# introlab/rtabmap

Measured on AMD Instinct MI355X. Metric: loop-closure candidates/sec (49k vocab, 100k signatures, 500 desc/frame), higher is better.
Workload: dtype f32; 1 GPU; SURF-64 fp32 brute-force 2-NN (49k words) + NNDR + TF-IDF likelihood (100000 signatures x 500 words, Zipf), 500 desc/frame, 1 frame/step; world_size_observed=1, collective_backend=none, parallelism=1 GPU, last_frame_top_candidate_ok=True

## Files before the change

### rtabmap_amd/csrc/bf16_filter_body.cuh

```cuda
#pragma once

constexpr int BF_KEEP = 2;
constexpr int BF_QW = 128;
constexpr int BF_NG = BF_QW / 32;
constexpr int BF_QB = BF_QW * MF_WAVES;
constexpr int BF_TILE_F = 32 * 64;
constexpr size_t BF_LDS_BYTES = (size_t)(MF_WAVES * 4 + 2) * BF_TILE_F * 4 + (size_t)MF_STRIP_TILES * 64 * 4;
typedef __bf16 bf16x8_t __attribute__((ext_vector_type(8)));

template <bool HI = false>
__device__ __forceinline__ void dma_tile_part(const float* __restrict__ base, int n_rows, int t, int lane, float* __restrict__ lds_slot,
                                              int i0, int i1) {
    for (int i = i0; i < i1; ++i) {
        const int p = i * 64 + lane;
        const int r = p >> 4, cpos = p & 15;
        const int c = cpos ^ (r & 15);
        if (HI && c >= 8) continue;
        const int row = min(t * 32 + r, n_rows - 1);
        __builtin_amdgcn_global_load_lds((const __attribute__((address_space(1))) void*)(base + (size_t)row * 64 + c * 4),
                                         (__attribute__((address_space(3))) void*)(lds_slot + i * 256), 16, 0, 0);
    }
}
typedef _Float16 f16x8_t __attribute__((ext_vector_type(8)));
template <int M>
// ... 449 lines not shown
            const int i = 2 * wave + j;
            if (half == 0 && (tile0 + i) * 32 + col >= lo_rows)
                asm volatile("ds_write_b32 %0, %1" ::"v"((uint32_t)(uintptr_t)(__attribute__((address_space(3))) void*)(s_aug + i * 64 + lane)),
                             "v"(__int_as_float(0x7f800000)) : "memory");
        }
        asm volatile("s_waitcnt lgkmcnt(0)" ::: "memory");
    }
    __builtin_amdgcn_s_barrier();
    MF_STAMP(1);
    int32_t k0[NG], k1[NG], k2[NG];
#pragma unroll
    for (int g = 0; g < NG; ++g) { k0[g] = MF_KEY_NONE; k1[g] = MF_KEY_NONE; k2[g] = MF_KEY_NONE; }
    f32x16 p0, p1;
    for (int t = tile0; t < tile1; ++t) {
        const int ti = t - tile0;
        if (ti == 2) {
            asm volatile("s_waitcnt vmcnt(0)" ::: "memory");
            __builtin_amdgcn_s_barrier();
        }
        uint4 ah[4], al[4];
        float aug;
        {
            const float* slot = s_dyn + (size_t)ti * BF_TILE_F;
            const uint32_t base = (uint32_t)(uintptr_t)(__attribute__((address_space(3))) const void*)(slot + col * 64);
            uint32_t addr[8];
            uint4 av[8];
#pragma unroll
            for (int v = 0; v < 4; ++v) {
                addr[v] = a_chunk_addr(base, 4 * half + v, col);
                addr[4 + v] = a_chunk_addr(base, 8 + 4 * half + v, col);
// ... 62 lines not shown
#pragma unroll
        for (int m = 0; m < 4; ++m)
            *reinterpret_cast<float4*>(xs + (size_t)ql * 32 + (((2 * m + half) ^ (ql & 7)) << 2)) = make_float4(c[g][4 * m], c[g][4 * m + 1], c[g][4 * m + 2], c[g][4 * m + 3]);
    }
    asm volatile("s_waitcnt lgkmcnt(0)" ::: "memory");
#pragma unroll 4
    for (int it = 0; it < QW / 8; ++it) {
        const int ql = it * 8 + (lane >> 3), ck = lane & 7;
        const int qi = q0 + ql;
        const float4 v = *reinterpret_cast<const float4*>(xs + (size_t)ql * 32 + ((ck ^ (ql & 7)) << 2));
        if (qi < nq) *reinterpret_cast<float4*>(x + (size_t)qi * ld + t * 32 + 4 * ck) = v;
    }
}

constexpr size_t BF_LDS_BYTES_P = (size_t)(MF_WAVES * 4 + 2) * BF_TILE_F * 4 + (size_t)2 * MF_STRIP_TILES * 64 * 4;
__device__ const float g_aug_inf[2] = {__builtin_inff(), 1.0f};
template <int M>
__device__ __forceinline__ void bf_request_strip(const float* __restrict__ vocab_bf, const float* __restrict__ row_norm, int n_rows, int bx,
                                                 int tiles_per_block, int n_tiles, int lane, int wave, int col, int half, float* slots, float* aug_dst) {
    constexpr int DPW = 8 / MF_WAVES;
    const int tile0 = bx * tiles_per_block;
    const int tile1 = min(tile0 + tiles_per_block, n_tiles);
#pragma unroll
    for (int i = 0; i < MF_STRIP_TILES; ++i) {
        const int t = min(tile0 + i, max(tile1 - 1, tile0));
        dma_tile_part<M == 1>(vocab_bf, n_rows, t, lane, slots + (size_t)i * BF_TILE_F, DPW * wave, DPW * wave + DPW);
    }
    if (wave == 0) {
#pragma unroll
        for (int i = 0; i < MF_STRIP_TILES; ++i) {
            const int t = min(tile0 + i, max(tile1 - 1, tile0));
            const float* src = t * 32 + col >= n_rows ? g_aug_inf + half : row_norm + 2 * (size_t)(t * 32 + col) + half;
            __builtin_amdgcn_global_load_lds((const __attribute__((address_space(1))) void*)src,
                                             (__attribute__((address_space(3))) void*)(aug_dst + i * 64), 4, 0, 0);
        }
    }
}
__device__ __forceinline__ void bf_wait_all_but_request(int wave) {
    constexpr int DPW = 8 / MF_WAVES;
    if (wave == 0) asm volatile("s_waitcnt vmcnt(%0)" :: "n"(MF_STRIP_TILES * DPW + MF_STRIP_TILES) : "memory");
    else asm volatile("s_waitcnt vmcnt(%0)" :: "n"(MF_STRIP_TILES * DPW) : "memory");
}
__device__ __forceinline__ void bf_lds_barrier() { asm volatile("s_waitcnt lgkmcnt(0)\n\ts_barrier" ::: "memory"); }
template <int M>
__device__ __forceinline__ void knn_bf16_filter_body_p(float* s_dyn, int bid, const float* __restrict__ vocab_bf, const float* __restrict__ row_norm,
                                                       int n_rows, const float* __restrict__ queries, int nq, int qpad,
                                                       int tiles_per_block, int n_blocks, int px, StripRecord* __restrict__ records, const SelfdistJob& sd,
                                                       const int32_t* __restrict__ n_lo = nullptr) {
    if (n_lo) n_rows = min(n_rows, max(n_lo[0], 1));
    constexpr int NG = BF_NG;
    constexpr int KH = 32;
    constexpr int NW = MF_WAVES;
    constexpr int QW = BF_QW;
    constexpr int DPW = 8 / NW;
    const int n_fwg = px * ((nq + BF_QB - 1) / BF_QB);
    if (bid >= n_fwg) { selfdist_tile(sd, bid - n_fwg, s_dyn); return; }
    const int fb = bid;
    const int bx0 = fb % px, by = fb / px;
    const int n_my = (n_blocks - bx0 + px - 1) / px;
    const int lane = threadIdx.x & 63;
    const int wave = __builtin_amdgcn_readfirstlane(threadIdx.x >> 6);
    const int col = lane & 31, half = lane >> 5;
    const int q0 = by * BF_QB + wave * QW;
    float* s_q = s_dyn + (size_t)wave * NG * BF_TILE_F;
    float* s_tile = s_dyn + (size_t)NW * NG * BF_TILE_F;
    float* s_aug = s_tile + 2 * BF_TILE_F;
    const int n_tiles = (n_rows + 31) / 32;
    {
        const int tile0 = bx0 * tiles_per_block;
        const int tile1 = min(tile0 + tiles_per_block, n_tiles);
#pragma unroll
        for (int g = 0; g < NG; ++g) dma_a_tile<KH>(queries, nq, q0 / 32 + g, lane, s_q + g * BF_TILE_F);
        float augs[MF_STRIP_TILES];
#pragma unroll
        for (int i = 0; i < MF_STRIP_TILES; ++i) {
            const int t = min(tile0 + i, max(tile1 - 1, tile0));
            augs[i] = t * 32 + col >= n_rows ? g_aug_inf[half] : row_norm[2 * (size_t)(t * 32 + col) + half];
        }
        if (tile0 < tile1) {
            dma_tile_part<M == 1>(vocab_bf, n_rows, tile0, lane, s_tile, DPW * wave, DPW * wave + DPW);
            dma_tile_part<M == 1>(vocab_bf, n_rows, min(tile0 + 1, tile1 - 1), lane, s_tile + BF_TILE_F, DPW * wave, DPW * wave + DPW);
        }
        asm volatile("s_waitcnt vmcnt(0)" ::: "memory");
        if (wave == 0) {
#pragma unroll
            for (int i = 0; i < MF_STRIP_TILES; ++i) s_aug[i * 64 + lane] = augs[i];
        }
    }
    uint4 bh[NG][4], bl[NG][4];
    float b_aug[NG];
#pragma unroll
    for (int g = 0; g < NG; ++g) split_query_group<M>(s_q + g * BF_TILE_F, col, half, bh[g], bl[g], b_aug[g]);
    __syncthreads();
    {
        const int tile0 = bx0 * tiles_per_block;
        const int tile1 = min(tile0 + tiles_per_block, n_tiles);
        for (int t = tile0 + 2; t < tile1; ++t)
            dma_tile_part<M == 1>(vocab_bf, n_rows, t, lane, s_dyn + (size_t)(t - tile0 - 2) * BF_TILE_F, DPW * wave, DPW * wave + DPW);
    }
    if (n_my > 1) bf_request_strip<M>(vocab_bf, row_norm, n_rows, bx0 + px, tiles_per_block, n_tiles, lane, wave, col, half,
                                   s_dyn + (size_t)8 * BF_TILE_F, s_aug + MF_STRIP_TILES * 64);
    for (int s = 0; s < n_my; ++s) {
        const int bx = bx0 + s * px;
        const int tile0 = bx * tiles_per_block;
        const int tile1 = min(tile0 + tiles_per_block, n_tiles);
        if (s > 0) {
            if (s + 1 < n_my) bf_wait_all_but_request(wave); else asm volatile("s_waitcnt vmcnt(0)" ::: "memory");
            bf_lds_barrier();
        }
        int32_t k0[NG], k1[NG], k2[NG];
#pragma unroll
        for (int g = 0; g < NG; ++g) { k0[g] = MF_KEY_NONE; k1[g] = MF_KEY_NONE; k2[g] = MF_KEY_NONE; }
        f32x16 p0, p1;
        const float* aug_s = s_aug + (s & 1) * (MF_STRIP_TILES * 64);
        for (int t = tile0; t < tile1; ++t) {
            const int ti = t - tile0;
            if (s == 0 && ti == 2) {
                if (n_my > 1) bf_wait_all_but_request(wave); else asm volatile("s_waitcnt vmcnt(0)" ::: "memory");
                bf_lds_barrier();
            }
            uint4 ah[4], al[4];
            float aug;
            {
                const float* slot = s == 0 ? (ti < 2 ? s_tile + ti * BF_TILE_F : s_dyn + (size_t)(ti - 2) * BF_TILE_F)
                                           : s_dyn + (size_t)(((s & 1) ? 8 : 0) + ti) * BF_TILE_F;
                const uint32_t base = (uint32_t)(uintptr_t)(__attribute__((address_space(3))) const void*)(slot + col * 64);
                uint32_t addr[8];
                uint4 av[8];
#pragma unroll
                for (int v = 0; v < 4; ++v) {
                    addr[v] = a_chunk_addr(base, 4 * half + v, col);
                    addr[4 + v] = a_chunk_addr(base, 8 + 4 * half + v, col);
                }
                lds_read_ops<M>(addr, av, (uint32_t)(uintptr_t)(__attribute__((address_space(3))) const void*)(aug_s + ti * 64 + lane), aug);
#pragma unroll
                for (int v = 0; v < 4; ++v) { ah[v] = av[v]; al[v] = av[4 + v]; }
            }
            tile_trip<M>(t == tile0, (uint32_t)ti, ah, al, aug, bh, bl, b_aug, p0, p1, k0, k1, k2);
        }
        if (tile0 < tile1) flush_pending(p0, p1, (uint32_t)(tile1 - 1 - tile0), k0, k1, k2);
#pragma unroll
        for (int g = 0; g < NG; ++g) merge_store_keys(k0[g], k1[g], k2[g], half, q0 + g * 32 + col, qpad, bx, records);
        if (s + 2 < n_my) {
            bf_lds_barrier();
            bf_request_strip<M>(vocab_bf, row_norm, n_rows, bx0 + (s + 2) * px, tiles_per_block, n_tiles, lane, wave, col, half,
                             s_dyn + (size_t)((s & 1) ? 8 : 0) * BF_TILE_F, s_aug + (s & 1) * (MF_STRIP_TILES * 64));
        }
    }
}
```

### rtabmap_amd/csrc/frame_pipeline.hip

```cpp
#include "engine_impl.h"

#include <algorithm>
#include <chrono>
#include <cstring>

using namespace lcd;

namespace {
struct FrameHostTimer {
    lcd_engine* h; std::chrono::steady_clock::time_point t0;
    explicit FrameHostTimer(lcd_engine* e) : h(e), t0(std::chrono::steady_clock::now()) {}
    ~FrameHostTimer() { h->frame_host_ns += std::chrono::duration_cast<std::chrono::nanoseconds>(std::chrono::steady_clock::now() - t0).count(); h->frame_calls += 1; }
};
struct HostLap {
    lcd_engine* h; std::chrono::steady_clock::time_point t;
    explicit HostLap(lcd_engine* e) : h(e), t(std::chrono::steady_clock::now()) {}
    void lap(int i) { const auto n = std::chrono::steady_clock::now(); h->host_prof[i] += std::chrono::duration_cast<std::chrono::nanoseconds>(n - t).count(); t = n; }
};
struct FrameShape { bool incremental, together; int ld, bw; };
inline FrameShape frame_shape(const lcd_frame_args& a) {
    const bool incremental = (a.flags & LCD_Q_INCREMENTAL) != 0;
    const int ld = (a.q + 63) / 64 * 64;
    return FrameShape{incremental, incremental && (a.flags & LCD_Q_NEW_WORDS_COMPARED) != 0, ld, ld / 32};
}
// ... 119 lines not shown
    PipeKnn& k = *kp;
    const lcd_frame_args& a = f.a;
    const int q = a.q;
    FramePipeline::FrameScratch& sc = h->pipe.scratch(f);
    const auto [incremental, together, ld, bw] = frame_shape(a);
    const int64_t rows_bound = f.chained ? h->applog.rows_ub(h->n_rows) : h->n_rows;
    const int64_t plan_rows = f.chained ? h->applog.rows_plan(f.vseq, h->n_rows) : h->n_rows;
    if (plan_rows > 0x7FFFFFF0ll) return h->fail(LCD_ERR_UNSUPPORTED, "lcd_frame_dev: more than 2^31 rows");
    k.plan = knn_bf16_plan_pipelined(q, (int)plan_rows, together ? knn_selfdist_wgs(q) : 0, h->filter_units);
    k.plan.f16 = h->f16();
    if (h->strip_tiles > 0 && plan_rows > 0) {
        const int n_tiles = (int)((plan_rows + 31) / 32);
        k.plan.tiles_per_block = h->strip_tiles; k.plan.n_blocks = (n_tiles + h->strip_tiles - 1) / h->strip_tiles; k.plan.one_strip = 1;
        k.plan.f16 = h->f16();
    }
    if (f_sh && !knn_bf16_persistent(k.plan) && plan_rows < (int64_t)SHADOW_ROW_BASE) {
        const FramePipeline::FrameScratch& ss = h->pipe.scratch(*f_sh);
        k.plan.n_shadow = 1;
        k.sh_bf = ss.d_shadow_bf.p; k.sh_norm = ss.d_shadow_norm.as<float>(); k.sh_rows = (f_sh->a.q + 63) / 64 * 64;
        k.sh_mask = ss.d_newmask.as<uint32_t>(); k.sh_q = f_sh->a.q;
        k.sh_ld = k.sh_rows;
        LCD_HIP(h, ring_reserve(h, f.set, &FramePipeline::FrameScratch::d_cross, (size_t)q * k.sh_ld * 4));
        k.sh_x = sc.d_cross.as<float>();
    }
    {
        size_t bytes = knn_bf16_partial_bytes(k.plan), want = 0;
        if (f.chained) {
            bytes = std::max(bytes, knn_bf16_partial_bytes(knn_bf16_plan_pipelined(q, (int)(rows_bound + 8 * (int64_t)q), together ? knn_selfdist_wgs(q) : 0, h->filter_units)));
            want = knn_bf16_partial_bytes(knn_bf16_plan_pipelined(q, (int)std::min<int64_t>(rows_bound + rows_bound / 2 + 65536, 0x7FFFFF00ll), together ? knn_selfdist_wgs(q) : 0, h->filter_units));
        }
        LCD_HIP(h, ring_reserve_grow(h, f.set, &FramePipeline::FrameScratch::d_partial2, bytes, want));
// ... 368 lines not shown
```

### rtabmap_amd/csrc/knn_mfma_kernels.hip

```cpp
#include <hip/hip_ext.h>
#include "lcd_kernels.h"
#include "rowpar_body.cuh"
#include "shard_body.cuh"
#include "frame_tail_body.cuh"
#include "score_body.cuh"

#include <algorithm>
#include <cstdlib>

namespace lcd {
namespace {

typedef float f32x16 __attribute__((ext_vector_type(16)));
constexpr int MF_BLOCK = 256;
constexpr int MF_WAVES = 4;
constexpr int MF_KEEP = 4;

__global__ void row_norm_kernel(const float* __restrict__ vocab, const int32_t* __restrict__ row_id, int first, int n, int dim,
                                float* __restrict__ aug, uint32_t* __restrict__ norm_max_bits) {
    const int r = first + blockIdx.x * blockDim.x + threadIdx.x;
    if (r >= first + n) return;
    float s = __int_as_float(0x7f800000);
    if (row_id[r] != 0) {
        s = 0.0f;
// ... 186 lines not shown
        top3_push32(k00, k01, k02, strip_key(p0[r], mask, base | (uint32_t)r));
        top3_push32(k10, k11, k12, strip_key(p1[r], mask, base | (uint32_t)r));
        __builtin_amdgcn_sched_barrier(0);
    }
}

constexpr int MF_NG = 4;
#ifdef LCD_MFMA_TIMING
__device__ unsigned long long g_mf_timing[4 * 4096];
#define MF_STAMP(i) do { if (lane == 0) g_mf_timing[4 * (((blockIdx.y * gridDim.x + blockIdx.x) & 1023) * MF_WAVES + wave) + (i)] = __builtin_amdgcn_s_memrealtime(); } while (0)
__device__ unsigned long long g_mf_timing2[8 * 4096];
#define MF_STAMP2(i) do { if (lane == 0 && (i) < 8) { g_mf_timing2[8 * (((blockIdx.y * gridDim.x + blockIdx.x) & 1023) * MF_WAVES + wave) + (i)] = __builtin_amdgcn_s_memrealtime(); } } while (0)
#else
#define MF_STAMP(i) do { } while (0)
#define MF_STAMP2(i) do { } while (0)
#endif

template <int DIM>
__global__ __launch_bounds__(MF_BLOCK, 1) void knn_mfma_filter_kernel(const float* __restrict__ vocab, const float* __restrict__ row_norm, int n_rows,
                                                                     const float* __restrict__ queries, int nq, int qpad, int tiles_per_block,
                                                                     uint64_t* __restrict__ partial_keys, uint32_t* __restrict__ partial_lmin) {
    constexpr int NG = MF_NG;
    constexpr int KH = DIM / 2;
    constexpr int QW = NG * 32;
    const int lane = threadIdx.x & 63;
    const int wave = __builtin_amdgcn_readfirstlane(threadIdx.x >> 6);
    const int col = lane & 31, half = lane >> 5;
    const int q0 = blockIdx.y * QW;
    MF_STAMP(0);

// ... 100 lines not shown
            for (int i = 0; i < MF_KEEP; ++i) partial_keys[((size_t)qi * gridDim.x + blockIdx.x) * MF_KEEP + i] = keep[i];
            partial_lmin[(size_t)qi * gridDim.x + blockIdx.x] = lmin;
        }
    }
    MF_STAMP(3);
}


#include "bf16_filter_body.cuh"

template <int M>
__global__ __launch_bounds__(256) void knn_bf16_filter_kernel_p(const float* __restrict__ vocab_bf, const float* __restrict__ row_norm, int n_rows,
                                                                const float* __restrict__ queries, int nq, int qpad, int tiles_per_block, int n_blocks,
                                                                int px, StripRecord* __restrict__ records, SelfdistJob sd) {
    extern __shared__ __attribute__((aligned(16))) float s_dyn_p[];
    knn_bf16_filter_body_p<M>(s_dyn_p, (int)blockIdx.x, vocab_bf, row_norm, n_rows, queries, nq, qpad, tiles_per_block, n_blocks, px, records, sd);
}

template <int M>
__global__ __launch_bounds__(MF_WAVES * 64) void knn_bf16_filter_kernel(const float* __restrict__ vocab_bf, const float* __restrict__ row_norm,
                                                                      int n_rows, const float* __restrict__ queries, int nq, int qpad,
                                                                      int tiles_per_block, int n_blocks, StripRecord* __restrict__ records,
                                                                      SelfdistJob sd) {
    extern __shared__ __attribute__((aligned(16))) float s_dyn_f[];
    knn_bf16_filter_body<M>(s_dyn_f, (int)blockIdx.x, vocab_bf, row_norm, n_rows, queries, nq, qpad, tiles_per_block, n_blocks, records, sd);
}

#include "rerank_body.cuh"

template <int DIM, int KEEP, bool LAST_KEY_BOUNDS, bool BF16>
__global__ __launch_bounds__(MF_BLOCK) void knn_mfma_rerank_kernel(KeptKeys<BF16> kk, int n_blocks, int nq,
// ... 34 lines not shown
__device__ unsigned long long g_a_timing[2 * 4096];
#define A_STAMP(i) do { __builtin_amdgcn_s_barrier(); if (threadIdx.x == 0 && blockIdx.x < 4096) g_a_timing[2 * blockIdx.x + (i)] = __builtin_amdgcn_s_memrealtime(); } while (0)
#else
#define A_STAMP(i) do { } while (0)
#endif
template <bool PERSISTENT, int M>
__device__ __forceinline__ void frame_a_body(float* s_dyn, const FilterArgs& f, int px, const TailRoles& tr, const ResolveArgs& r, const FwArgs& a,
                                             const RetireArgs& ret, const QSplitArgs& qs) {
    const int bid = (int)blockIdx.x;
    const int n_front = tr.has_resolve + tr.has_register;
    A_STAMP(0);
    if (bid < tr.has_resolve) { frame_resolve_part<PIPE_BLOCK>((uint32_t*)s_dyn, r, 0, 1 + tr.n_redo); A_STAMP(1); return; }
    if (bid < n_front) { frame_register_part<PIPE_BLOCK>((uint32_t*)s_dyn, a, ret); A_STAMP(1); return; }
    const int after_strips = n_front + tr.n_filter_wgs;
    if (bid >= after_strips && bid < after_strips + tr.n_sh_wgs) {
        if constexpr (!PERSISTENT) shadow_scores_body<M>(s_dyn, bid - after_strips, f.sh_bf, f.sh_norm, f.sh_rows, f.qsplit, f.qnorm, f.nq, f.qpad, f.sh_x, f.sh_ld);
        A_STAMP(1);
        return;
    }
    const int after_filter = after_strips + tr.n_sh_wgs;
    if (bid >= after_filter && bid < after_filter + tr.n_q_wgs) { qsplit_body(qs, bid - after_filter); A_STAMP(1); return; }
    if (bid >= after_filter + tr.n_q_wgs) { frame_resolve_part<PIPE_BLOCK>((uint32_t*)s_dyn, r, bid - after_filter - tr.n_q_wgs + 1, 1 + tr.n_redo); A_STAMP(1); return; }
    for (int i = 0; i < f.delay; ++i) __builtin_amdgcn_s_sleep(1);
    if constexpr (PERSISTENT)
        knn_bf16_filter_body_p<M>(s_dyn, bid - n_front, f.vocab_bf, f.row_norm, f.n_rows, f.queries, f.nq, f.qpad, f.tiles_per_block, f.n_blocks, px,
                               f.records, f.sd, f.n_lo);
    else
        knn_bf16_filter_body_q<M>(s_dyn, bid - n_front, f.vocab_bf, f.row_norm, f.n_rows, f.qsplit, f.qnorm, f.nq, f.qpad, f.tiles_per_block, f.n_blocks,
                               f.records, f.sd, f.n_lo);
    A_STAMP(1);
}
template <int M>
__global__ __launch_bounds__(PIPE_BLOCK, 2) void frame_a_kernel(FilterArgs f, TailRoles tr, ResolveArgs r, FwArgs a, RetireArgs ret, QSplitArgs qs) {
    extern __shared__ __attribute__((aligned(16))) float s_dyn_a[];
    frame_a_body<false, M>(s_dyn_a, f, 0, tr, r, a, ret, qs);
}
template <int M>
__global__ __launch_bounds__(PIPE_BLOCK) void frame_a_kernel_p(FilterArgs f, int px, TailRoles tr, ResolveArgs r, FwArgs a, RetireArgs ret, QSplitArgs qs) {
    extern __shared__ __attribute__((aligned(16))) float s_dyn_ap[];
    frame_a_body<true, M>(s_dyn_ap, f, px, tr, r, a, ret, qs);
}
// ... 224 lines not shown
}
size_t knn_bf16_partial_bytes(const MfmaPlan& p) {
    const size_t nb = (size_t)(p.n_blocks > 0 ? p.n_blocks : 1);
    static_assert(sizeof(StripRecord) == 16, "one 16-byte request per (block, query)");
    return nb * p.qpad * sizeof(StripRecord);
}
hipError_t launch_vocab_bf16(const void* vocab, int first, int n, int dim, void* bf, hipStream_t s, int f16) {
    if (n <= 0) return hipSuccess;
    if (dim != 64) return hipErrorInvalidValue;
    vocab_bf16_kernel<<<(n * 16 + 255) / 256, 256, 0, s>>>((const float*)vocab, first, n, (uint32_t*)bf, f16);
    return hipGetLastError();
}
static int bf16_persistent_px(const MfmaPlan& p) {
    const int cus = p.filter_units >= 0 ? p.filter_units : g_plan_cus - p.other_wgs;
    const int qchunks = (p.q + BF_QB - 1) / BF_QB;
    if (p.one_strip || cus <= 0 || qchunks <= 0 || p.n_blocks * qchunks <= (p.filter_units >= 0 ? g_plan_cus : cus)) return 0;
    const int px_max = cus / qchunks > 0 ? cus / qchunks : 1;
    const int rounds = (p.n_blocks + px_max - 1) / px_max;
    return (p.n_blocks + rounds - 1) / rounds;
}
bool knn_bf16_persistent(const MfmaPlan& p) { return p.q > 0 && bf16_persistent_px(p) > 0; }
MfmaPlan knn_bf16_plan_pipelined(int q, int n_rows, int n_tile_wgs, int filter_units) {
    MfmaPlan p = knn_bf16_plan(q, n_rows, n_tile_wgs);
    p.filter_units = filter_units;
    if (bf16_persistent_px(p) == 0) return p;
    if (filter_units >= 0) {
        p = knn_bf16_plan(q, n_rows, 2 + n_tile_wgs);
        p.filter_units = filter_units;
        return p;
    }
    const int n_tiles = (n_rows + 31) / 32;
    const int qchunks = (q + BF_QB - 1) / BF_QB;
    const int slots = (2 * (g_plan_cus - p.other_wgs) - 16) / qchunks;
    if (slots > 0 && n_tiles <= slots * MF_STRIP_TILES) {
        int tpb = (n_tiles + slots - 1) / slots;
        if (tpb < 1) tpb = 1;
        p.tiles_per_block = tpb;
        p.n_blocks = (n_tiles + tpb - 1) / tpb;
        p.one_strip = 1;
        return p;
// ... 181 lines not shown
        if (p.n_shadow > 0 && k.sh_bf && k.sh_norm && k.sh_rows > 0 && k.sh_x) { f.sh_bf = (const float*)k.sh_bf; f.sh_norm = k.sh_norm; f.sh_rows = k.sh_rows; f.sh_x = k.sh_x; f.sh_ld = k.sh_ld; }
        f.vocab_bf = (const float*)k.vocab_bf; f.row_norm = k.row_norm; f.n_rows = p.n_rows; f.queries = (const float*)k.queries; f.nq = p.q; f.qpad = p.qpad;
        f.tiles_per_block = p.tiles_per_block; f.n_blocks = p.n_blocks; f.records = (StripRecord*)k.partial; f.n_lo = k.n_lo;
        f.qsplit = (const uint4*)k.qsplit; f.qnorm = k.qnorm;
        if (k.cb.selfdist) {
            f.sd.queries = (const float*)k.queries; f.sd.nq = p.q; f.sd.out = const_cast<float*>(k.cb.selfdist); f.sd.ld = k.cb.ld; f.sd.n_tiles = f.sd.n_self = selfdist_tiles(p.q);
        }
        if (opt.cross_frames && k.cross && k.cross_cols && k.cross_ncols > 0 && p.q > 0) {
            f.sd.queries = (const float*)k.queries; f.sd.nq = p.q;
            f.sd.other = (const float*)k.cross_cols; f.sd.n_other = k.cross_ncols; f.sd.xout = k.cross; f.sd.xld = k.cross_ld;
            f.sd.n_tiles += ((p.q + 63) / 64) * ((k.cross_ncols + 63) / 64);
        }
    }
    f.delay = opt.filter_delay;
    const int px = p.q > 0 ? bf16_persistent_px(p) : 0;
    if (px == 0 && p.q > 0 && (!f.qsplit || !f.qnorm)) return hipErrorInvalidValue;
    if (p.n_shadow > 0 && (px > 0 || !f.sh_x)) return hipErrorInvalidValue;
    TailRoles tr;
    tr.n_filter_wgs = p.q > 0 ? f.sd.n_tiles + (px > 0 ? px : p.n_blocks) * ((p.q + BF_QB - 1) / BF_QB) : 0;
    tr.n_sh_wgs = (p.q > 0 && p.n_shadow > 0) ? ((f.sh_rows + 31) / 32) * ((p.q + BF_QB - 1) / BF_QB) : 0;
    tr.has_resolve = resolve ? 1 : 0; tr.has_register = reg ? 1 : 0; tr.n_redo = resolve ? resolve->n_redo : 0;
    QSplitArgs qs{};
    if (qsp) { qs = *qsp; qs.n_wgs = std::min((qs.qpad * 8 + PIPE_BLOCK - 1) / PIPE_BLOCK, 32); if (qs.n_wgs < 1) qs.n_wgs = 1; }
    tr.n_q_wgs = qsp ? qs.n_wgs : 0;
    const int grid = tr.n_filter_wgs + tr.n_sh_wgs + tr.has_resolve + tr.has_register + tr.n_redo + tr.n_q_wgs;
    if (grid == 0) return hipSuccess;
    const size_t lds = px > 0 ? BF_LDS_BYTES_P : BF_LDS_BYTES_Q;
    if ((resolve && resolve->shmem_resolve > lds) || (reg && reg->shmem + (size_t)reg->a.n * 4 > lds)) return hipErrorInvalidValue;
    ResolveArgs r{}; FwArgs a{}; RetireArgs ret{};
    if (resolve) { r = resolve->r; r.ap.lds_bytes = (int)lds; }
    if (reg) { a = reg->a; ret = reg->ret; }
    const bool timed = ev_begin != nullptr && ev_end != nullptr;
    const bool f16 = kp ? p.f16 != 0 : opt.f16 != 0;
    if (px > 0) {
        static const hipError_t attrp0 = hipFuncSetAttribute(reinterpret_cast<const void*>(&frame_a_kernel_p<0>),
                                                             hipFuncAttributeMaxDynamicSharedMemorySize, (int)BF_LDS_BYTES_P);
        static const hipError_t attrp1 = hipFuncSetAttribute(reinterpret_cast<const void*>(&frame_a_kernel_p<1>),
                                                             hipFuncAttributeMaxDynamicSharedMemorySize, (int)BF_LDS_BYTES_P);
        (void)attrp0; (void)attrp1;
        auto kern = f16 ? frame_a_kernel_p<1> : frame_a_kernel_p<0>;
        if (timed) hipExtLaunchKernelGGL(kern, dim3(grid), dim3(PIPE_BLOCK), (uint32_t)BF_LDS_BYTES_P, s, ev_begin, ev_end, 0u, f, px, tr, r, a, ret, qs);
        else kern<<<grid, PIPE_BLOCK, BF_LDS_BYTES_P, s>>>(f, px, tr, r, a, ret, qs);
    } else {
        auto kern = f16 ? frame_a_kernel<1> : frame_a_kernel<0>;
        if (timed) hipExtLaunchKernelGGL(kern, dim3(grid), dim3(PIPE_BLOCK), (uint32_t)BF_LDS_BYTES_Q, s, ev_begin, ev_end, 0u, f, tr, r, a, ret, qs);
        else kern<<<grid, PIPE_BLOCK, BF_LDS_BYTES_Q, s>>>(f, tr, r, a, ret, qs);
    }
    return hipGetLastError();
}


static long long g_b_routes[8];
hipError_t launch_frame_b(const PipeKnn* k, const ScoreArgs* score, int score_wgs, hipStream_t s, hipEvent_t ev_begin, hipEvent_t ev_end,
                          const AppendRowsArgs* app, const PipeOpts& opt) {
    RerankArgs rk{};
    int n_rerank = 0;
    if (k) {
// ... 47 lines not shown
}

extern "C" int lcd_debug_launch_b_routes(long long* out8, int reset) {
    if (out8) for (int i = 0; i < 8; ++i) out8[i] = lcd::g_b_routes[i];
    if (reset) for (int i = 0; i < 8; ++i) lcd::g_b_routes[i] = 0;
    return 0;
}

extern "C" int lcd_debug_frame_plan(int q, int n_rows, int new_words_compared, int* out) {
    if (q <= 0 || n_rows <= 0 || !out) return -1;
    const int tiles = new_words_compared ? lcd::knn_selfdist_wgs(q) : 0;
    const lcd::MfmaPlan p = lcd::knn_bf16_plan_pipelined(q, n_rows, tiles, -1);
    out[0] = p.tiles_per_block; out[1] = p.n_blocks; out[2] = lcd::bf16_persistent_px(p); out[3] = tiles; out[4] = (q + lcd::BF_QB - 1) / lcd::BF_QB;
    return 0;
}

extern "C" int lcd_debug_wide_mfma_plan(int q, int n_rows, int dim, int units, int* out9) {
    lcd::WidePlan p;
    if (!out9 || !lcd::knn_wide_mfma_plan(q, n_rows, dim, units, &p)) return -1;
    out9[0] = p.tiles_per_block; out9[1] = p.n_blocks; out9[2] = p.n_qblocks; out9[3] = p.group_q; out9[4] = p.qpad;
    out9[5] = (int)(lcd::knn_wide_partial_bytes(p) / 4); out9[6] = lcd::MF_STRIP_TILES;
    out9[7] = (p.tiles_per_block + lcd::MF_STRIP_TILES - 1) / lcd::MF_STRIP_TILES; out9[8] = p.n_wgs;
    return 0;
}

#ifdef LCD_SCORE_TIMING
extern "C" int lcd_debug_score_timing_pipe(unsigned long long* out, int n_words) {
    if (hipDeviceSynchronize() != hipSuccess) return -1;
    return (int)hipMemcpyFromSymbol(out, HIP_SYMBOL(lcd::g_score_timing), (size_t)n_words * 8);
}
// ... 11 lines not shown
```

### rtabmap_amd/csrc/lcd_kernels.h

```cpp
#pragma once
#include <hip/hip_runtime.h>
#include <stdint.h>

namespace lcd {

static const uint64_t KEY_NONE = ~0ull;

struct KnnPlan {
    int q;
    int qpad;
    int n_rows;
    int rows_per_block;
    int n_blocks;
};
KnnPlan knn_plan(int q, int n_rows, int dim_bytes);
size_t knn_partial_bytes(const KnnPlan& p);

hipError_t launch_knn2_partial(int dtype, int dim, const void* vocab, const int32_t* row_id, const void* queries,
                               const KnnPlan& p, uint64_t* partial, hipStream_t s);
hipError_t launch_knn2_merge(int dtype, const KnnPlan& p, const uint64_t* partial, const int32_t* row_id,
                             int32_t* out_row, int32_t* out_word, float* out_dist, hipStream_t s);
hipError_t launch_knn2_merge_selfdist_hamming(const KnnPlan& p, const uint64_t* partial, const int32_t* row_id, int32_t* out_row, int32_t* out_word,
                                              float* out_dist, const void* queries, int dim_bytes, float* selfdist, int ld, int have_index, uint32_t* bits,
                                              int bw, hipStream_t s);
// ... 49 lines not shown
struct RowparArgs {
    int enabled = 0;
    const float* vocab = nullptr; const int32_t* row_id = nullptr; int n_rows = 0;
    const int32_t* n_rows_dev = nullptr;
    const float* queries = nullptr; const int32_t* fail_list = nullptr;
    unsigned long long* partial = nullptr;
    int32_t* out_row = nullptr; int32_t* out_word = nullptr; float* out_dist = nullptr;
    CandBits cb;
};

struct MfmaPlan {
    int q, qpad, n_rows, tiles_per_block, n_blocks;
    int filter_units = -1;
    int other_wgs = 0;
    int one_strip = 0;
    int f16 = 0;
    int n_shadow = 0;
};
constexpr uint32_t SHADOW_ROW_BASE = 1u << 30;
bool knn_mfma_supported(int dtype, int dim);
void knn_set_compute_units(int cus);
bool knn_bf16_persistent(const MfmaPlan& p);
MfmaPlan knn_mfma_plan(int q, int n_rows);
MfmaPlan knn_bf16_plan_pipelined(int q, int n_rows, int n_tile_wgs, int filter_units);
size_t knn_mfma_partial_bytes(const MfmaPlan& p);
hipError_t launch_row_norms(const void* vocab, const int32_t* row_id, int first, int n, int dim, float* norm, uint32_t* norm_max_bits,
                            hipStream_t s);
hipError_t launch_norm_tombstone(float* norm, const int32_t* rows, int n, hipStream_t s);
hipError_t launch_vocab_tail(float* norm, void* bf, long long first, long long n, hipStream_t s);
size_t knn_rowpar_partial_bytes(int n_rows, int q);
// ... 75 lines not shown
```

Baseline: 4.043 billion candidates/s.

## Use presplit queries in persistent bf16 filter and enable shadow with persistent path

The persistent bf16 filter body gains a PRESPLIT mode that loads pre-split query fragments and norms from global memory instead of staging queries in LDS and splitting them per workgroup. This frees the query LDS region so vocab tiles can sit directly in slots, and the LDS budget shrinks (BF_LDS_BYTES_PQ). Shadow scoring is now allowed alongside the persistent path, and a new units-based planner picks tiles_per_block when persistence is not chosen. It also adds timing stamp macros that compile away by default. The risks are a changed strip count and grid shape that may alter load balance.

```diff
diff --git a/rtabmap_amd/csrc/bf16_filter_body.cuh b/rtabmap_amd/csrc/bf16_filter_body.cuh
--- a/rtabmap_amd/csrc/bf16_filter_body.cuh
+++ b/rtabmap_amd/csrc/bf16_filter_body.cuh
@@ -487,6 +487,7 @@
     f32x16 p0, p1;
     for (int t = tile0; t < tile1; ++t) {
         const int ti = t - tile0;
+        MF_STAMP2T(ti);
         if (ti == 2) {
             asm volatile("s_waitcnt vmcnt(0)" ::: "memory");
             __builtin_amdgcn_s_barrier();
@@ -579,7 +580,17 @@
 }
 
 constexpr size_t BF_LDS_BYTES_P = (size_t)(MF_WAVES * 4 + 2) * BF_TILE_F * 4 + (size_t)2 * MF_STRIP_TILES * 64 * 4;
+constexpr size_t BF_LDS_BYTES_PQ = (size_t)2 * MF_STRIP_TILES * BF_TILE_F * 4 + (size_t)2 * MF_STRIP_TILES * 64 * 4;
 __device__ const float g_aug_inf[2] = {__builtin_inff(), 1.0f};
+__device__ __forceinline__ void bf_request_aug(const float* __restrict__ row_norm, int n_rows, int tile0, int tile1, int col, int half, float* aug_dst) {
+#pragma unroll
+    for (int i = 0; i < MF_STRIP_TILES; ++i) {
+        const int t = min(tile0 + i, max(tile1 - 1, tile0));
+        const float* src = t * 32 + col >= n_rows ? g_aug_inf + half : row_norm + 2 * (size_t)(t * 32 + col) + half;
+        __builtin_amdgcn_global_load_lds((const __attribute__((address_space(1))) void*)src,
+                                         (__attribute__((address_space(3))) void*)(aug_dst + i * 64), 4, 0, 0);
+    }
+}
 template <int M>
 __device__ __forceinline__ void bf_request_strip(const float* __restrict__ vocab_bf, const float* __restrict__ row_norm, int n_rows, int bx,
                                                  int tiles_per_block, int n_tiles, int lane, int wave, int col, int half, float* slots, float* aug_dst) {
@@ -591,15 +602,7 @@
         const int t = min(tile0 + i, max(tile1 - 1, tile0));
         dma_tile_part<M == 1>(vocab_bf, n_rows, t, lane, slots + (size_t)i * BF_TILE_F, DPW * wave, DPW * wave + DPW);
     }
-    if (wave == 0) {
-#pragma unroll
-        for (int i = 0; i < MF_STRIP_TILES; ++i) {
-            const int t = min(tile0 + i, max(tile1 - 1, tile0));
-            const float* src = t * 32 + col >= n_rows ? g_aug_inf + half : row_norm + 2 * (size_t)(t * 32 + col) + half;
-            __builtin_amdgcn_global_load_lds((const __attribute__((address_space(1))) void*)src,
-                                             (__attribute__((address_space(3))) void*)(aug_dst + i * 64), 4, 0, 0);
-        }
-    }
+    if (wave == 0) bf_request_aug(row_norm, n_rows, tile0, tile1, col, half, aug_dst);
 }
 __device__ __forceinline__ void bf_wait_all_but_request(int wave) {
     constexpr int DPW = 8 / MF_WAVES;
@@ -607,9 +610,9 @@
     else asm volatile("s_waitcnt vmcnt(%0)" :: "n"(MF_STRIP_TILES * DPW) : "memory");
 }
 __device__ __forceinline__ void bf_lds_barrier() { asm volatile("s_waitcnt lgkmcnt(0)\n\ts_barrier" ::: "memory"); }
-template <int M>
+template <int M, bool PRESPLIT>
 __device__ __forceinline__ void knn_bf16_filter_body_p(float* s_dyn, int bid, const float* __restrict__ vocab_bf, const float* __restrict__ row_norm,
-                                                       int n_rows, const float* __restrict__ queries, int nq, int qpad,
+                                                       int n_rows, const float* __restrict__ queries, const uint4* qsplit, const float* qnorm, int nq, int qpad,
                                                        int tiles_per_block, int n_blocks, int px, StripRecord* __restrict__ records, const SelfdistJob& sd,
                                                        const int32_t* __restrict__ n_lo = nullptr) {
     if (n_lo) n_rows = min(n_rows, max(n_lo[0], 1));
@@ -620,6 +623,7 @@
     constexpr int DPW = 8 / NW;
     const int n_fwg = px * ((nq + BF_QB - 1) / BF_QB);
     if (bid >= n_fwg) { selfdist_tile(sd, bid - n_fwg, s_dyn); return; }
+    __builtin_amdgcn_s_waitcnt(0x0F70);
     const int fb = bid;
     const int bx0 = fb % px, by = fb / px;
     const int n_my = (n_blocks - bx0 + px - 1) / px;
@@ -629,50 +633,73 @@
     const int q0 = by * BF_QB + wave * QW;
     float* s_q = s_dyn + (size_t)wave * NG * BF_TILE_F;
     float* s_tile = s_dyn + (size_t)NW * NG * BF_TILE_F;
-    float* s_aug = s_tile + 2 * BF_TILE_F;
+    float* s_aug = PRESPLIT ? s_dyn + (size_t)2 * MF_STRIP_TILES * BF_TILE_F : s_tile + 2 * BF_TILE_F;
+    MF_STAMP(0);
     const int n_tiles = (n_rows + 31) / 32;
-    {
+    uint4 bh[NG][4], bl[NG][4];
+    float b_aug[NG];
+    if constexpr (PRESPLIT) {
         const int tile0 = bx0 * tiles_per_block;
         const int tile1 = min(tile0 + tiles_per_block, n_tiles);
-#pragma unroll
-        for (int g = 0; g < NG; ++g) dma_a_tile<KH>(queries, nq, q0 / 32 + g, lane, s_q + g * BF_TILE_F);
-        float augs[MF_STRIP_TILES];
-#pragma unroll
-        for (int i = 0; i < MF_STRIP_TILES; ++i) {
-            const int t = min(tile0 + i, max(tile1 - 1, tile0));
-            augs[i] = t * 32 + col >= n_rows ? g_aug_inf[half] : row_norm[2 * (size_t)(t * 32 + col) + half];
-        }
-        if (tile0 < tile1) {
-            dma_tile_part<M == 1>(vocab_bf, n_rows, tile0, lane, s_tile, DPW * wave, DPW * wave + DPW);
-            dma_tile_part<M == 1>(vocab_bf, n_rows, min(tile0 + 1, tile1 - 1), lane, s_tile + BF_TILE_F, DPW * wave, DPW * wave + DPW);
-        }
+        const int tile_last = max(tile1 - 1, tile0);
+        dma_tile_part<M == 1>(vocab_bf, n_rows, tile0, lane, s_dyn, DPW * wave, DPW * wave + DPW);
+        dma_tile_part<M == 1>(vocab_bf, n_rows, min(tile0 + 1, tile_last), lane, s_dyn + BF_TILE_F, DPW * wave, DPW * wave + DPW);
+        if (wave == 0) bf_request_aug(row_norm, n_rows, tile0, tile1, col, half, s_aug);
+        const int grp0 = q0 >> 5, n_grp = qpad >> 5;
+#pragma unroll
+        for (int g = 0; g < NG; ++g)
+            load_group_presplit(qsplit, qnorm, min(grp0 + g, n_grp - 1), qpad, lane, col, half, bh[g], bl[g], b_aug[g]);
+        asm volatile("" : "+v"(b_aug[NG - 1]) : : "memory");
         asm volatile("s_waitcnt vmcnt(0)" ::: "memory");
-        if (wave == 0) {
-#pragma unroll
-            for (int i = 0; i < MF_STRIP_TILES; ++i) s_aug[i * 64 + lane] = augs[i];
-        }
-    }
-    uint4 bh[NG][4], bl[NG][4];
-    float b_aug[NG];
-#pragma unroll
-    for (int g = 0; g < NG; ++g) split_query_group<M>(s_q + g * BF_TILE_F, col, half, bh[g], bl[g], b_aug[g]);
-    __syncthreads();
-    {
-        const int tile0 = bx0 * tiles_per_block;
-        const int tile1 = min(tile0 + tiles_per_block, n_tiles);
         for (int t = tile0 + 2; t < tile1; ++t)
-            dma_tile_part<M == 1>(vocab_bf, n_rows, t, lane, s_dyn + (size_t)(t - tile0 - 2) * BF_TILE_F, DPW * wave, DPW * wave + DPW);
+            dma_tile_part<M == 1>(vocab_bf, n_rows, t, lane, s_dyn + (size_t)(t - tile0) * BF_TILE_F, DPW * wave, DPW * wave + DPW);
+    } else {
+        {
+            const int tile0 = bx0 * tiles_per_block;
+            const int tile1 = min(tile0 + tiles_per_block, n_tiles);
+#pragma unroll
+            for (int g = 0; g < NG; ++g) dma_a_tile<KH>(queries, nq, q0 / 32 + g, lane, s_q + g * BF_TILE_F);
+            float augs[MF_STRIP_TILES];
+#pragma unroll
+            for (int i = 0; i < MF_STRIP_TILES; ++i) {
+                const int t = min(tile0 + i, max(tile1 - 1, tile0));
+                augs[i] = t * 32 + col >= n_rows ? g_aug_inf[half] : row_norm[2 * (size_t)(t * 32 + col) + half];
+            }
+            if (tile0 < tile1) {
+                dma_tile_part<M == 1>(vocab_bf, n_rows, tile0, lane, s_tile, DPW * wave, DPW * wave + DPW);
+                dma_tile_part<M == 1>(vocab_bf, n_rows, min(tile0 + 1, tile1 - 1), lane, s_tile + BF_TILE_F, DPW * wave, DPW * wave + DPW);
+            }
+            asm volatile("s_waitcnt vmcnt(0)" ::: "memory");
+            if (wave == 0) {
+#pragma unroll
+                for (int i = 0; i < MF_STRIP_TILES; ++i) s_aug[i * 64 + lane] = augs[i];
+            }
+        }
+#pragma unroll
+        for (int g = 0; g < NG; ++g) split_query_group<M>(s_q + g * BF_TILE_F, col, half, bh[g], bl[g], b_aug[g]);
+        __syncthreads();
+        {
+            const int tile0 = bx0 * tiles_per_block;
+            const int tile1 = min(tile0 + tiles_per_block, n_tiles);
+            for (int t = tile0 + 2; t < tile1; ++t)
+                dma_tile_part<M == 1>(vocab_bf, n_rows, t, lane, s_dyn + (size_t)(t - tile0 - 2) * BF_TILE_F, DPW * wave, DPW * wave + DPW);
+        }
     }
     if (n_my > 1) bf_request_strip<M>(vocab_bf, row_norm, n_rows, bx0 + px, tiles_per_block, n_tiles, lane, wave, col, half,
                                    s_dyn + (size_t)8 * BF_TILE_F, s_aug + MF_STRIP_TILES * 64);
+    if constexpr (PRESPLIT) __builtin_amdgcn_s_barrier();
+    MF_STAMP(1);
     for (int s = 0; s < n_my; ++s) {
         const int bx = bx0 + s * px;
         const int tile0 = bx * tiles_per_block;
         const int tile1 = min(tile0 + tiles_per_block, n_tiles);
         if (s > 0) {
+            MF_STAMP2W(5 + s);
             if (s + 1 < n_my) bf_wait_all_but_request(wave); else asm volatile("s_waitcnt vmcnt(0)" ::: "memory");
+            if (s == 1) MF_STAMPW(2);
             bf_lds_barrier();
         }
+        MF_STAMP2S(2 * s);
         int32_t k0[NG], k1[NG], k2[NG];
 #pragma unroll
         for (int g = 0; g < NG; ++g) { k0[g] = MF_KEY_NONE; k1[g] = MF_KEY_NONE; k2[g] = MF_KEY_NONE; }
@@ -684,11 +711,12 @@
                 if (n_my > 1) bf_wait_all_but_request(wave); else asm volatile("s_waitcnt vmcnt(0)" ::: "memory");
                 bf_lds_barrier();
             }
+            if (s == 1) MF_STAMP2T(ti);
             uint4 ah[4], al[4];
             float aug;
             {
-                const float* slot = s == 0 ? (ti < 2 ? s_tile + ti * BF_TILE_F : s_dyn + (size_t)(ti - 2) * BF_TILE_F)
-                                           : s_dyn + (size_t)(((s & 1) ? 8 : 0) + ti) * BF_TILE_F;
+                const float* slot = !PRESPLIT && s == 0 ? (ti < 2 ? s_tile + ti * BF_TILE_F : s_dyn + (size_t)(ti - 2) * BF_TILE_F)
+                                                        : s_dyn + (size_t)(((s & 1) ? 8 : 0) + ti) * BF_TILE_F;
                 const uint32_t base = (uint32_t)(uintptr_t)(__attribute__((address_space(3))) const void*)(slot + col * 64);
                 uint32_t addr[8];
                 uint4 av[8];
@@ -706,10 +734,12 @@
         if (tile0 < tile1) flush_pending(p0, p1, (uint32_t)(tile1 - 1 - tile0), k0, k1, k2);
 #pragma unroll
         for (int g = 0; g < NG; ++g) merge_store_keys(k0[g], k1[g], k2[g], half, q0 + g * 32 + col, qpad, bx, records);
+        MF_STAMP2S(2 * s + 1);
         if (s + 2 < n_my) {
             bf_lds_barrier();
             bf_request_strip<M>(vocab_bf, row_norm, n_rows, bx0 + (s + 2) * px, tiles_per_block, n_tiles, lane, wave, col, half,
                              s_dyn + (size_t)((s & 1) ? 8 : 0) * BF_TILE_F, s_aug + (s & 1) * (MF_STRIP_TILES * 64));
         }
     }
-}
+    MF_STAMP(3);
+}
diff --git a/rtabmap_amd/csrc/frame_pipeline.hip b/rtabmap_amd/csrc/frame_pipeline.hip
--- a/rtabmap_amd/csrc/frame_pipeline.hip
+++ b/rtabmap_amd/csrc/frame_pipeline.hip
@@ -157,7 +157,7 @@
         k.plan.tiles_per_block = h->strip_tiles; k.plan.n_blocks = (n_tiles + h->strip_tiles - 1) / h->strip_tiles; k.plan.one_strip = 1;
         k.plan.f16 = h->f16();
     }
-    if (f_sh && !knn_bf16_persistent(k.plan) && plan_rows < (int64_t)SHADOW_ROW_BASE) {
+    if (f_sh && plan_rows < (int64_t)SHADOW_ROW_BASE) {
         const FramePipeline::FrameScratch& ss = h->pipe.scratch(*f_sh);
         k.plan.n_shadow = 1;
         k.sh_bf = ss.d_shadow_bf.p; k.sh_norm = ss.d_shadow_norm.as<float>(); k.sh_rows = (f_sh->a.q + 63) / 64 * 64;
diff --git a/rtabmap_amd/csrc/knn_mfma_kernels.hip b/rtabmap_amd/csrc/knn_mfma_kernels.hip
--- a/rtabmap_amd/csrc/knn_mfma_kernels.hip
+++ b/rtabmap_amd/csrc/knn_mfma_kernels.hip
@@ -224,6 +224,20 @@
 #else
 #define MF_STAMP(i) do { } while (0)
 #define MF_STAMP2(i) do { } while (0)
+#endif
+#if defined(LCD_MFMA_TIMING) && LCD_MFMA_TIMING + 0 == 3
+#define MF_STAMP2S(i) do { } while (0)
+#define MF_STAMP2T(i) MF_STAMP2(i)
+#else
+#define MF_STAMP2S(i) MF_STAMP2(i)
+#define MF_STAMP2T(i) do { } while (0)
+#endif
+#if defined(LCD_MFMA_TIMING) && LCD_MFMA_TIMING + 0 == 2
+#define MF_STAMP2W(i) MF_STAMP2(i)
+#define MF_STAMPW(i) MF_STAMP(i)
+#else
+#define MF_STAMP2W(i) do { } while (0)
+#define MF_STAMPW(i) do { } while (0)
 #endif
 
 template <int DIM>
@@ -354,7 +368,8 @@
                                                                 const float* __restrict__ queries, int nq, int qpad, int tiles_per_block, int n_blocks,
                                                                 int px, StripRecord* __restrict__ records, SelfdistJob sd) {
     extern __shared__ __attribute__((aligned(16))) float s_dyn_p[];
-    knn_bf16_filter_body_p<M>(s_dyn_p, (int)blockIdx.x, vocab_bf, row_norm, n_rows, queries, nq, qpad, tiles_per_block, n_blocks, px, records, sd);
+    knn_bf16_filter_body_p<M, false>(s_dyn_p, (int)blockIdx.x, vocab_bf, row_norm, n_rows, queries, nullptr, nullptr, nq, qpad, tiles_per_block, n_blocks, px,
+                                     records, sd);
 }
 
 template <int M>
@@ -419,7 +434,7 @@
     if (bid < n_front) { frame_register_part<PIPE_BLOCK>((uint32_t*)s_dyn, a, ret); A_STAMP(1); return; }
     const int after_strips = n_front + tr.n_filter_wgs;
     if (bid >= after_strips && bid < after_strips + tr.n_sh_wgs) {
-        if constexpr (!PERSISTENT) shadow_scores_body<M>(s_dyn, bid - after_strips, f.sh_bf, f.sh_norm, f.sh_rows, f.qsplit, f.qnorm, f.nq, f.qpad, f.sh_x, f.sh_ld);
+        shadow_scores_body<M>(s_dyn, bid - after_strips, f.sh_bf, f.sh_norm, f.sh_rows, f.qsplit, f.qnorm, f.nq, f.qpad, f.sh_x, f.sh_ld);
         A_STAMP(1);
         return;
     }
@@ -428,8 +443,8 @@
     if (bid >= after_filter + tr.n_q_wgs) { frame_resolve_part<PIPE_BLOCK>((uint32_t*)s_dyn, r, bid - after_filter - tr.n_q_wgs + 1, 1 + tr.n_redo); A_STAMP(1); return; }
     for (int i = 0; i < f.delay; ++i) __builtin_amdgcn_s_sleep(1);
     if constexpr (PERSISTENT)
-        knn_bf16_filter_body_p<M>(s_dyn, bid - n_front, f.vocab_bf, f.row_norm, f.n_rows, f.queries, f.nq, f.qpad, f.tiles_per_block, f.n_blocks, px,
-                               f.records, f.sd, f.n_lo);
+        knn_bf16_filter_body_p<M, true>(s_dyn, bid - n_front, f.vocab_bf, f.row_norm, f.n_rows, f.queries, f.qsplit, f.qnorm, f.nq, f.qpad, f.tiles_per_block,
+                                        f.n_blocks, px, f.records, f.sd, f.n_lo);
     else
         knn_bf16_filter_body_q<M>(s_dyn, bid - n_front, f.vocab_bf, f.row_norm, f.n_rows, f.qsplit, f.qnorm, f.nq, f.qpad, f.tiles_per_block, f.n_blocks,
                                f.records, f.sd, f.n_lo);
@@ -684,7 +699,7 @@
 static int bf16_persistent_px(const MfmaPlan& p) {
     const int cus = p.filter_units >= 0 ? p.filter_units : g_plan_cus - p.other_wgs;
     const int qchunks = (p.q + BF_QB - 1) / BF_QB;
-    if (p.one_strip || cus <= 0 || qchunks <= 0 || p.n_blocks * qchunks <= (p.filter_units >= 0 ? g_plan_cus : cus)) return 0;
+    if (p.one_strip || cus <= 0 || qchunks <= 0 || p.n_blocks * qchunks <= (p.filter_units >= 0 && !p.units_plan ? g_plan_cus : cus)) return 0;
     const int px_max = cus / qchunks > 0 ? cus / qchunks : 1;
     const int rounds = (p.n_blocks + px_max - 1) / px_max;
     return (p.n_blocks + rounds - 1) / rounds;
@@ -693,7 +708,18 @@
 MfmaPlan knn_bf16_plan_pipelined(int q, int n_rows, int n_tile_wgs, int filter_units) {
     MfmaPlan p = knn_bf16_plan(q, n_rows, n_tile_wgs);
     p.filter_units = filter_units;
-    if (bf16_persistent_px(p) == 0) return p;
+    if (bf16_persistent_px(p) == 0) {
+        if (filter_units <= 0) return p;
+        const int n_tiles = (n_rows + 31) / 32;
+        const int qchunks = (q + BF_QB - 1) / BF_QB;
+        const int per_q = filter_units / qchunks > 0 ? filter_units / qchunks : 1;
+        const int w = std::max((n_tiles + per_q - 1) / per_q, 1);
+        const int rounds = (w + MF_STRIP_TILES - 1) / MF_STRIP_TILES;
+        p.tiles_per_block = std::min(std::max((w + rounds - 1) / rounds, 1), (int)MF_STRIP_TILES);
+        p.n_blocks = n_tiles > 0 ? (n_tiles + p.tiles_per_block - 1) / p.tiles_per_block : 0;
+        p.units_plan = 1;
+        return p;
+    }
     if (filter_units >= 0) {
         p = knn_bf16_plan(q, n_rows, 2 + n_tile_wgs);
         p.filter_units = filter_units;
@@ -905,8 +931,8 @@
     }
     f.delay = opt.filter_delay;
     const int px = p.q > 0 ? bf16_persistent_px(p) : 0;
-    if (px == 0 && p.q > 0 && (!f.qsplit || !f.qnorm)) return hipErrorInvalidValue;
-    if (p.n_shadow > 0 && (px > 0 || !f.sh_x)) return hipErrorInvalidValue;
+    if (p.q > 0 && (!f.qsplit || !f.qnorm)) return hipErrorInvalidValue;
+    if (p.n_shadow > 0 && !f.sh_x) return hipErrorInvalidValue;
     TailRoles tr;
     tr.n_filter_wgs = p.q > 0 ? f.sd.n_tiles + (px > 0 ? px : p.n_blocks) * ((p.q + BF_QB - 1) / BF_QB) : 0;
     tr.n_sh_wgs = (p.q > 0 && p.n_shadow > 0) ? ((f.sh_rows + 31) / 32) * ((p.q + BF_QB - 1) / BF_QB) : 0;
@@ -916,7 +942,7 @@
     tr.n_q_wgs = qsp ? qs.n_wgs : 0;
     const int grid = tr.n_filter_wgs + tr.n_sh_wgs + tr.has_resolve + tr.has_register + tr.n_redo + tr.n_q_wgs;
     if (grid == 0) return hipSuccess;
-    const size_t lds = px > 0 ? BF_LDS_BYTES_P : BF_LDS_BYTES_Q;
+    const size_t lds = px > 0 ? BF_LDS_BYTES_PQ : BF_LDS_BYTES_Q;
     if ((resolve && resolve->shmem_resolve > lds) || (reg && reg->shmem + (size_t)reg->a.n * 4 > lds)) return hipErrorInvalidValue;
     ResolveArgs r{}; FwArgs a{}; RetireArgs ret{};
     if (resolve) { r = resolve->r; r.ap.lds_bytes = (int)lds; }
@@ -925,13 +951,13 @@
     const bool f16 = kp ? p.f16 != 0 : opt.f16 != 0;
     if (px > 0) {
         static const hipError_t attrp0 = hipFuncSetAttribute(reinterpret_cast<const void*>(&frame_a_kernel_p<0>),
-                                                             hipFuncAttributeMaxDynamicSharedMemorySize, (int)BF_LDS_BYTES_P);
+                                                             hipFuncAttributeMaxDynamicSharedMemorySize, (int)BF_LDS_BYTES_PQ);
         static const hipError_t attrp1 = hipFuncSetAttribute(reinterpret_cast<const void*>(&frame_a_kernel_p<1>),
-                                                             hipFuncAttributeMaxDynamicSharedMemorySize, (int)BF_LDS_BYTES_P);
+                                                             hipFuncAttributeMaxDynamicSharedMemorySize, (int)BF_LDS_BYTES_PQ);
         (void)attrp0; (void)attrp1;
         auto kern = f16 ? frame_a_kernel_p<1> : frame_a_kernel_p<0>;
-        if (timed) hipExtLaunchKernelGGL(kern, dim3(grid), dim3(PIPE_BLOCK), (uint32_t)BF_LDS_BYTES_P, s, ev_begin, ev_end, 0u, f, px, tr, r, a, ret, qs);
-        else kern<<<grid, PIPE_BLOCK, BF_LDS_BYTES_P, s>>>(f, px, tr, r, a, ret, qs);
+        if (timed) hipExtLaunchKernelGGL(kern, dim3(grid), dim3(PIPE_BLOCK), (uint32_t)BF_LDS_BYTES_PQ, s, ev_begin, ev_end, 0u, f, px, tr, r, a, ret, qs);
+        else kern<<<grid, PIPE_BLOCK, BF_LDS_BYTES_PQ, s>>>(f, px, tr, r, a, ret, qs);
     } else {
         auto kern = f16 ? frame_a_kernel<1> : frame_a_kernel<0>;
         if (timed) hipExtLaunchKernelGGL(kern, dim3(grid), dim3(PIPE_BLOCK), (uint32_t)BF_LDS_BYTES_Q, s, ev_begin, ev_end, 0u, f, tr, r, a, ret, qs);
@@ -1009,6 +1035,13 @@
     out[0] = p.tiles_per_block; out[1] = p.n_blocks; out[2] = lcd::bf16_persistent_px(p); out[3] = tiles; out[4] = (q + lcd::BF_QB - 1) / lcd::BF_QB;
     return 0;
 }
+extern "C" int lcd_debug_frame_plan_units(int q, int n_rows, int new_words_compared, int units, int* out) {
+    if (q <= 0 || n_rows <= 0 || !out) return -1;
+    const int tiles = new_words_compared ? lcd::knn_selfdist_wgs(q) : 0;
+    const lcd::MfmaPlan p = lcd::knn_bf16_plan_pipelined(q, n_rows, tiles, units);
+    out[0] = p.tiles_per_block; out[1] = p.n_blocks; out[2] = lcd::bf16_persistent_px(p); out[3] = tiles; out[4] = (q + lcd::BF_QB - 1) / lcd::BF_QB;
+    return 0;
+}
 
 extern "C" int lcd_debug_wide_mfma_plan(int q, int n_rows, int dim, int units, int* out9) {
     lcd::WidePlan p;
diff --git a/rtabmap_amd/csrc/lcd_kernels.h b/rtabmap_amd/csrc/lcd_kernels.h
--- a/rtabmap_amd/csrc/lcd_kernels.h
+++ b/rtabmap_amd/csrc/lcd_kernels.h
@@ -87,6 +87,7 @@
     int filter_units = -1;
     int other_wgs = 0;
     int one_strip = 0;
+    int units_plan = 0;
     int f16 = 0;
     int n_shadow = 0;
 };
```

Result: no change. 4.104 billion candidates/s (median of 6 runs) (+1.5%).
